# G-U-N/a-PyTorch-Tutorial-to-Class-Incremental-Learning

Measured on AMD Instinct MI355X. Metric: imgs/sec/node (CIFAR-100 B0-Inc10 ResNet-18 WA+KD step), higher is better.
Workload: dtype bf16; 1 GPU; model=resnet18, global_batch=128, input_size=32, kd=True, hip_graph=True, parallelism=dp1

## Files before the change

cilfw/_hip_ops.py:

```python

import ctypes
import os

import torch

_LIB_PATH = os.path.join(os.path.dirname(os.path.abspath(__file__)),
                         "_hip_lib.so")
if not os.path.exists(_LIB_PATH):
    raise ImportError(f"cilfw HIP library not built: {_LIB_PATH}")
_lib = ctypes.CDLL(_LIB_PATH)

_DEBUG = os.environ.get("CILFW_SYNC_DEBUG") == "1"

c_vp = ctypes.c_void_p
c_i = ctypes.c_int
c_l = ctypes.c_long
c_f = ctypes.c_float

_lib.cilfw_sync.restype = c_i
_lib.cilfw_error_string.restype = ctypes.c_char_p
_lib.cilfw_error_string.argtypes = [c_i]

_PROTOS = {
    "cilfw_conv2d_fwd": [c_vp] * 4 + [c_i] * 12 + [c_vp, c_vp],
    "cilfw_conv2d_bwd_data": [c_vp] * 4 + [c_i] * 12 + [c_vp] * 5 + [c_i, c_vp],
    "cilfw_conv2d_bwd_weight": [c_vp] * 5 + [c_i] * 13 + [c_vp],
    "cilfw_fill_mtable": [c_vp] + [c_i] * 4 + [c_vp],
    "cilfw_im2col_smallc": [c_vp] * 3 + [c_i] * 11 + [c_vp],
    "cilfw_bn_apply_only": [c_vp] * 7 + [c_l, c_i, c_i, c_vp],
    "cilfw_bn_fwd": [c_vp] * 11 + [c_i, c_l, c_i, c_f, c_f, c_i, c_i, c_vp],
    "cilfw_bn_bwd": [c_vp] * 11 + [c_vp, c_i] + [c_l, c_i, c_i, c_i, c_vp],
    "cilfw_add_relu_fwd": [c_vp] * 3 + [c_l, c_vp],
    "cilfw_add_relu_bwd": [c_vp] * 3 + [c_l, c_vp],
    "cilfw_downsample_a_fwd": [c_vp] * 2 + [c_i] * 4 + [c_vp],
    "cilfw_downsample_a_bwd": [c_vp] * 2 + [c_i] * 4 + [c_vp],
    "cilfw_gap_fwd": [c_vp] * 2 + [c_i] * 3 + [c_vp],
    "cilfw_gap_bwd": [c_vp] * 2 + [c_i] * 3 + [c_vp],
    "cilfw_conv2d_bwd_data_sub": [c_vp] * 4 + [c_i] * 12 + [c_vp],
    "cilfw_parity_scatter": [c_vp] * 2 + [c_i] * 8 + [c_vp],
    "cilfw_stride_gather": [c_vp] * 2 + [c_i] * 7 + [c_vp],
    "cilfw_stride_scatter": [c_vp] * 2 + [c_i] * 7 + [c_vp],
    "cilfw_maxpool_fwd": [c_vp] * 3 + [c_i] * 9 + [c_vp],
    "cilfw_maxpool_bwd": [c_vp] * 3 + [c_i] * 9 + [c_vp],
    "cilfw_linear_fwd": [c_vp] * 5 + [c_i] * 4 + [c_vp],
    "cilfw_linear_dx": [c_vp] * 4 + [c_i] * 4 + [c_vp],
    "cilfw_linear_dw": [c_vp] * 5 + [c_i] * 4 + [c_vp],
    "cilfw_ce_fwd": [c_vp] * 5 + [c_i, c_i, c_f, c_vp],
    "cilfw_ce_bwd": [c_vp] * 4 + [c_i, c_i, c_f, c_vp],
    "cilfw_kd_fwd": [c_vp] * 6 + [c_i, c_i, c_f, c_vp],
    "cilfw_kd_bwd": [c_vp] * 4 + [c_i, c_i, c_f, c_vp],
    "cilfw_wa_loss_fwd": [c_vp] * 8 + [c_i] * 3 + [c_f] * 3 + [c_vp],
    "cilfw_wa_loss_bwd": [c_vp] * 6 + [c_i] * 3 + [c_f] * 3 + [c_vp],
    "cilfw_sgd_step": [c_vp] * 4 + [c_l, c_vp, c_f, c_f, c_vp],
    "cilfw_topk_correct": [c_vp] * 3 + [c_i] * 3 + [c_vp],
    "cilfw_herding_select": [c_vp] * 3 + [c_i] * 3 + [c_vp],
    "cilfw_herding_select_batch": [c_vp] * 6 + [c_i] * 3 + [c_vp],
    "cilfw_crop_resize": [c_vp] * 7 + [c_i] * 7 + [c_vp],
    "cilfw_crop_resize_ragged": [c_vp] * 9 + [c_i] * 5 + [c_vp],
    "cilfw_nme_prototypes": [c_vp] * 3 + [c_i] * 2 + [c_vp],
    "cilfw_nme_topk": [c_vp] * 6 + [c_i] * 4 + [c_vp],
}
for _name, _args in _PROTOS.items():
    _fn = getattr(_lib, _name)
    _fn.argtypes = _args
    _fn.restype = None

_lib.cilfw_conv2d_bwd_data.restype = c_i

for _name, _n in [("cilfw_linear_ksplit", 3),
                  ("cilfw_conv2d_fwd_ksplit", 7),
                  ("cilfw_conv2d_bwd_data_ksplit", 7),
                  ("cilfw_conv2d_bwd_data_can_fuse_bn", 8),
                  ("cilfw_conv2d_bwd_data_bn_gy", 3),
                  ("cilfw_conv2d_bwd_weight_nslices", 7),
                  ("cilfw_conv2d_fwd_route", 8),
                  ("cilfw_conv2d_bwd_data_route", 9),
                  ("cilfw_conv2d_bwd_weight_route", 8)]:
    _fn = getattr(_lib, _name)
    _fn.argtypes = [c_i] * _n
    _fn.restype = c_i

_FWD_ROUTES = ("v1_bk32", "v1_bk64", "v2_bn64", "v2_bn128")
_BWD_DATA_ROUTES = ("s2_fused", "v2", "v1_bk32", "v1_bk64")
_BWD_WEIGHT_ROUTES = ("v2", "v1_fast", "v1_generic")


def _stream():
    return c_vp(torch.cuda.current_stream().cuda_stream)


# ... 47 lines not shown
        H, W_, stride = (H - 1) // stride + 1, (W_ - 1) // stride + 1, 1
    ks = _lib.cilfw_conv2d_bwd_data_ksplit(N, H, W_, C, K, R, S)
    return _BWD_DATA_ROUTES[_lib.cilfw_conv2d_bwd_data_route(
        N, H, W_, C, K, R, S, stride, ks)], ks


def _stem_im2col_dw(C, K, R, S):
    use_im2col = (os.environ.get("CILFW_STEM_IM2COL") == "1"
                  or (R * S >= 25
                      and os.environ.get("CILFW_STEM_IM2COL") != "0"))
    return C < 16 and R * S > 1 and K % 16 == 0 and use_im2col


def conv2d_bwd_weight_route(N, C, K, R, S, Ho, Wo, accum=False):
    if _stem_im2col_dw(C, K, R, S):
        N, C, R, S, Ho, Wo = N * Ho * Wo, (C * R * S + 15) // 16 * 16, 1, 1, \
            1, 1
        accum = False
    ns = _lib.cilfw_conv2d_bwd_weight_nslices(N, C, K, R, S, Ho, Wo)
    return _BWD_WEIGHT_ROUTES[_lib.cilfw_conv2d_bwd_weight_route(
        N, C, K, R, S, Ho, Wo, 1 if accum else 0)], ns


def conv2d_fwd(x, w, stride, pad, want_bn_parts=False):
    _bf16(x, "conv2d_fwd.x")
    _bf16(w, "conv2d_fwd.w")
    N, H, W_, C = x.shape
    R, S, Cw, K = w.shape
    assert Cw == C
    assert K % 8 == 0, "conv kernels vector-stage over output channels (K%8==0)"
    Ho = (H + 2 * pad - R) // stride + 1
    Wo = (W_ + 2 * pad - S) // stride + 1
    if C < 16 and R * S > 1 and K % 16 == 0 \
            and os.environ.get("CILFW_STEM_IM2COL") == "1":
        CRS = C * R * S
        CRSpad = (CRS + 15) // 16 * 16
        col, Ho, Wo = _stem_cols(x, stride, pad, R, S, CRSpad)
        M = N * Ho * Wo
        wpad = torch.zeros(CRSpad, K, dtype=torch.bfloat16, device=x.device)
        wpad[:CRS] = w.reshape(CRS, K)
        y = torch.empty(M, K, dtype=torch.bfloat16, device=x.device)
        ks = _lib.cilfw_conv2d_fwd_ksplit(M, CRSpad, K, 1, 1, 1, 1)
        ws = (torch.empty(ks * M * K, dtype=torch.float32, device=x.device)
              if ks > 1 else None)
        _lib.cilfw_conv2d_fwd(_ptr(col), _ptr(wpad), _ptr(y), _ptr(ws),
                              c_i(M), c_i(1), c_i(1), c_i(CRSpad), c_i(K),
                              c_i(1), c_i(1), c_i(1), c_i(0), c_i(1), c_i(1),
                              c_i(ks), _ptr(None), _stream())
        _check("conv2d_fwd_stem")
        return y.view(N, Ho, Wo, K), None
    y = torch.empty(N, Ho, Wo, K, dtype=torch.bfloat16, device=x.device)
    ks = _lib.cilfw_conv2d_fwd_ksplit(N, C, K, R, S, Ho, Wo)
    ws = (torch.empty(ks * N * Ho * Wo * K, dtype=torch.float32,
                      device=x.device) if ks > 1 else None)
    parts = None
    if want_bn_parts and ks == 1 \
            and _FWD_ROUTES[_lib.cilfw_conv2d_fwd_route(
                N, C, K, R, S, Ho, Wo, ks)].startswith("v2_") \
            and os.environ.get("CILFW_CONV_BN_FUSE", "1") != "0":
        gy = (N * Ho * Wo + 127) // 128
        parts = torch.empty(gy * 2 * K, dtype=torch.float32,
                            device=x.device)
    _lib.cilfw_conv2d_fwd(_ptr(x), _ptr(w), _ptr(y), _ptr(ws), c_i(N),
                          c_i(H), c_i(W_), c_i(C), c_i(K), c_i(R), c_i(S),
                          c_i(stride), c_i(pad), c_i(Ho), c_i(Wo), c_i(ks),
                          _ptr(parts), _stream())
    _check("conv2d_fwd")
    return y, parts


def conv2d_bwd_data(dy, w, stride, pad, H, W_, bn_meta=None):
    _bf16(dy, "conv2d_bwd_data.dy")
    N, Ho, Wo, K = dy.shape
    R, S, C, Kw = w.shape
    assert Kw == K
    if R == 1 and S == 1 and stride > 1:
        dxs = conv2d_bwd_data(dy, w, 1, 0, Ho, Wo)
        dx = torch.empty(N, H, W_, C, dtype=torch.bfloat16, device=dy.device)
        _lib.cilfw_stride_scatter(_ptr(dxs), _ptr(dx), c_i(N), c_i(H),
                                  c_i(W_), c_i(C), c_i(stride), c_i(Ho),
                                  c_i(Wo), _stream())
        _check("stride_scatter")
        return (dx, None) if bn_meta is not None else dx
    dx = torch.empty(N, H, W_, C, dtype=torch.bfloat16, device=dy.device)
    ks = _lib.cilfw_conv2d_bwd_data_ksplit(N, H, W_, C, K, R, S)
    ws = (torch.empty(ks * N * H * W_ * C, dtype=torch.float32,
                      device=dy.device) if ks > 1 else None)
    parts = None
    if (bn_meta is not None
            and _lib.cilfw_conv2d_bwd_data_can_fuse_bn(
                N, H, W_, C, K, R, S, stride)):
# ... 567 lines not shown
```

cilfw/csrc/common.h:

```cpp
#pragma once
#include <hip/hip_runtime.h>
#include <stdint.h>

#define WAVE 64
#define DEV __device__ __forceinline__

typedef __attribute__((ext_vector_type(8))) short bf16x8;
typedef __attribute__((ext_vector_type(4))) float f32x4;
typedef unsigned short bf16_t;

DEV float bf2f(bf16_t v) {
  union { uint32_t u; float f; } x;
  x.u = ((uint32_t)v) << 16;
  return x.f;
}

DEV bf16_t f2bf(float f) {
  union { uint32_t u; float f; } x;
  x.f = f;
  uint32_t u = x.u;
  uint32_t r = (u + 0x7fffu + ((u >> 16) & 1u)) >> 16;
  if ((u & 0x7f800000u) == 0x7f800000u && (u & 0x7fffffu)) r = (u >> 16) | 1u;
  return (bf16_t)r;
}

DEV int cdiv_i(int a, int b) { return (a + b - 1) / b; }
static inline int cdiv(int a, int b) { return (a + b - 1) / b; }

struct FragIdx {
  int half;
  int quad;
};
DEV FragIdx frag_idx() {
  int lane = threadIdx.x & (WAVE - 1);
  return {lane & 15, lane >> 4};
}
```

cilfw/csrc/conv.hip:

```cpp

#include "common.h"

#define BM 128
#define BN 64
#define NTHREADS 256

struct ConvGeom {
  int N, H, W, C, K, R, S, stride, pad, pad2, Ho, Wo;
  unsigned long long m_howo, m_wo;
  unsigned long long m_ck, m_s;
};

static inline unsigned long long magic40(int d) {
  return d > 0 ? ((1ULL << 40) / (unsigned)d + 1) : 0;
}

DEV unsigned mdiv40(unsigned n, unsigned long long m) {
  return (unsigned)(((unsigned long long)n * m) >> 40);
}

__global__ __launch_bounds__(NTHREADS)
void reduce_slabs_bf16_kernel(const float* __restrict__ ws,
                              bf16_t* __restrict__ out, int ns, long len) {
  long i0 = ((long)blockIdx.x * NTHREADS + threadIdx.x) * 4;
// ... 17 lines not shown

__global__ __launch_bounds__(NTHREADS)
void reduce_slabs_f32_kernel(const float* __restrict__ ws,
                             float* __restrict__ out, int ns, long len,
                             int accum) {
  long i0 = ((long)blockIdx.x * NTHREADS + threadIdx.x) * 4;
  if (i0 >= len) return;
  if (i0 + 4 <= len) {
    float4 acc = *(const float4*)&ws[i0];
    for (int s = 1; s < ns; ++s) {
      float4 v = *(const float4*)&ws[(long)s * len + i0];
      acc.x += v.x; acc.y += v.y; acc.z += v.z; acc.w += v.w;
    }
    if (accum) {
      float4 o = *(const float4*)&out[i0];
      acc.x += o.x; acc.y += o.y; acc.z += o.z; acc.w += o.w;
    }
    *(float4*)&out[i0] = acc;
  } else {
    for (long i = i0; i < len; ++i) {
      float a = ws[i];
      for (int s = 1; s < ns; ++s) a += ws[(long)s * len + i];
      out[i] = accum ? out[i] + a : a;
    }
  }
}


__device__ __forceinline__ int4 masked_i4(int4 v, bool ok) {
  int4 z{0, 0, 0, 0};
  return ok ? v : z;
}

template <int BKT, int BMX = BM, int BNX = BN, bool FAST = true>
__global__ __launch_bounds__(NTHREADS)
void conv2d_fwd_kernel(const bf16_t* __restrict__ x,
                       const bf16_t* __restrict__ w,
                       bf16_t* __restrict__ y, float* __restrict__ ws,
                       ConvGeom g, int M, int CRS, int nk, int fast_a,
                       int ksplit) {
  constexpr int NQ = BKT / 32;
  constexpr int LPX = BKT + 8;
  constexpr int NR = BMX / 128;
  constexpr int MR = BMX / 32;
  constexpr int NRC = BNX / 32;
  __shared__ bf16_t lds[2 * BMX * LPX + 2 * BNX * LPX];
// ... 794 lines not shown
  bf16_t* dst = &col[(long)m * CRSpad + rs * g.C];
  for (int c = 0; c < g.C; ++c) dst[c] = src[c];
}

__global__ __launch_bounds__(NTHREADS)
void fill_mtable_kernel(int* __restrict__ mt, int M, int HoWo, int Wo,
                        int stride) {
  int m = blockIdx.x * NTHREADS + threadIdx.x;
  if (m >= M) return;
  int n = m / HoWo;
  int rem = m - n * HoWo;
  int ho = rem / Wo;
  int wo = rem - ho * Wo;
  mt[m] = (n << 20) | ((ho * stride) << 10) | (wo * stride);
}



#define V2BK 64
#define V2_A_ELEMS (BM * V2BK)
#define V2_B_ELEMS (4 * V2BK * 16)
#define V2_BUF (V2_A_ELEMS + V2_B_ELEMS)

template <int BNX2 = BN>
__global__ __launch_bounds__(NTHREADS)
void conv2d_fwd_v2_kernel(const bf16_t* __restrict__ x,
                          const bf16_t* __restrict__ w,
                          bf16_t* __restrict__ y, float* __restrict__ ws,
                          const bf16_t* __restrict__ zpage, ConvGeom g,
                          int M, int CRS, int nk, int ksplit,
                          float* __restrict__ bn_parts) {
  constexpr int NGRP = BNX2 / 16;
  constexpr int NRC = BNX2 / 32;
  constexpr int BEL = NGRP * V2BK * 16;
  constexpr int BUFE = V2_A_ELEMS + BEL;
  __shared__ bf16_t lds[2 * BUFE];
  const int m0 = blockIdx.x * BM;
  const int n0 = blockIdx.y * BNX2;
  const int t = threadIdx.x;
  const int wv = t >> 6, lane = t & 63;
  const int wr = wv >> 1, wc = wv & 1;
  const int steps = (nk + ksplit - 1) / ksplit;
  const int kt0 = blockIdx.z * steps;
  const int kt1 = min(kt0 + steps, nk);
  const int nsteps = kt1 - kt0;

  int achunk[4], ar[4], as_[4], ac[4];
  bool mok[4];
  int an[4], ahb[4], awb[4];
#pragma unroll
  for (int i = 0; i < 4; ++i) {
    int row = wv * 32 + i * 8 + (lane >> 3);
    achunk[i] = (lane & 7) ^ (row & 7);
    int m = m0 + row;
// ... 90 lines not shown
    for (int q = 0; q < 2; ++q) {
      const int kb = fq * 8 + q * 32;
#pragma unroll
      for (int mr = 0; mr < 4; ++mr) {
        int row = wr * 64 + mr * 16 + fh;
        int kcol = kb ^ ((row & 7) << 3);
        bf16x8 afr = *(const bf16x8*)&As[row * V2BK + kcol];
        if (q == 0 && mr == 0) {
          asm volatile("s_waitcnt lgkmcnt(0)" ::: "memory");
          __builtin_amdgcn_sched_barrier(0);
          __builtin_amdgcn_s_setprio(1);
        }
#pragma unroll
        for (int nr = 0; nr < NRC; ++nr)
          acc[mr][nr] = __builtin_amdgcn_mfma_f32_16x16x32_bf16(
              afr, bfr[q][nr], acc[mr][nr], 0, 0, 0);
      }
    }
    __builtin_amdgcn_s_setprio(0);
    asm volatile("s_waitcnt vmcnt(0)" ::: "memory");
    __builtin_amdgcn_s_barrier();
  }

#pragma unroll
  for (int mr = 0; mr < 4; ++mr)
#pragma unroll
    for (int nr = 0; nr < NRC; ++nr)
#pragma unroll
      for (int r = 0; r < 4; ++r) {
        int row = m0 + wr * 64 + mr * 16 + fq * 4 + r;
        int col = n0 + wc * (16 * NRC) + nr * 16 + fh;
        if (row < M && col < g.K) {
          if (ksplit > 1)
            ws[((long)blockIdx.z * M + row) * g.K + col] = acc[mr][nr][r];
          else
            y[(long)row * g.K + col] = f2bf(acc[mr][nr][r]);
        }
      }

  if (bn_parts != nullptr) {
    __syncthreads();
    float* red = (float*)lds;
#pragma unroll
    for (int nr = 0; nr < NRC; ++nr) {
      float s1 = 0.f, s2 = 0.f;
#pragma unroll
      for (int mr = 0; mr < 4; ++mr)
#pragma unroll
        for (int r = 0; r < 4; ++r) {
          int row = m0 + wr * 64 + mr * 16 + fq * 4 + r;
          float v = (row < M) ? bf2f(f2bf(acc[mr][nr][r])) : 0.f;
          s1 += v;
          s2 += v * v;
        }
      int cl = wc * (16 * NRC) + nr * 16 + fh;
      red[((wv * 4 + fq) * BNX2 + cl) * 2] = s1;
// ... 415 lines not shown
      bn128 = e ? atoi(e) : 1;
    }
    static int min3x3 = -2;
    if (min3x3 == -2) {
      const char* e = getenv("CILFW_CONV_V2_BN128_MIN3X3");
      min3x3 = e ? atoi(e) : -1;
    }
    int shape_ok = (R == 1 && S == 1) || (min3x3 >= 0 && M >= min3x3);
    if (bn128 && K % 128 == 0 && shape_ok &&
        cdiv(M, BM) * cdiv(K, 128) * ksplit >= 256)
      return FWD_V2_BN128;
    return FWD_V2_BN64;
  }
  int use64 = bm == BM && (CRS >= bk64_min_crs()) &&
              (cdiv(M, BM) * cdiv(K, BN) * ksplit < bk64_max_blocks());
  return use64 ? FWD_V1_BK64 : FWD_V1_BK32;
}

int cilfw_conv2d_fwd_route(int N, int C, int K, int R, int S, int Ho, int Wo,
                           int ksplit) {
  return fwd_route(N * Ho * Wo, C, K, R, S, ksplit, 1);
}

void cilfw_conv2d_fwd(const void* x, const void* w, void* y, void* ws,
                      int N, int H, int W, int C, int K, int R, int S,
                      int stride, int pad, int Ho, int Wo, int ksplit,
                      void* bn_parts, void* stream) {
  ConvGeom g{N, H, W, C, K, R, S, stride, pad, pad, Ho, Wo,
             0, 0, magic40(C), magic40(S)};
  int M = N * Ho * Wo;
  int CRS = C * R * S;
  int fast_a = (C % 16 == 0);
  void* zp = fwd_v2_eligible(C) ? zpage_ptr() : nullptr;
  int route = fwd_route(M, C, K, R, S, ksplit, zp != nullptr);
  if (route == FWD_V2_BN128 || route == FWD_V2_BN64) {
    int nk2 = cdiv(CRS, V2BK);
    int bn2 = route == FWD_V2_BN128 ? 128 : BN;
    dim3 grid2(cdiv(M, BM), cdiv(K, bn2), ksplit);
    float* parts = (float*)(ksplit > 1 ? nullptr : bn_parts);
    if (route == FWD_V2_BN128)
      hipLaunchKernelGGL(conv2d_fwd_v2_kernel<128>, grid2, dim3(NTHREADS),
                         0, (hipStream_t)stream, (const bf16_t*)x,
                         (const bf16_t*)w, (bf16_t*)y, (float*)ws,
                         (const bf16_t*)zp, g, M, CRS, nk2, ksplit, parts);
    else
      hipLaunchKernelGGL(conv2d_fwd_v2_kernel<BN>, grid2, dim3(NTHREADS), 0,
                         (hipStream_t)stream, (const bf16_t*)x,
                         (const bf16_t*)w, (bf16_t*)y, (float*)ws,
                         (const bf16_t*)zp, g, M, CRS, nk2, ksplit, parts);
    if (ksplit > 1) {
      long len = (long)M * K;
      hipLaunchKernelGGL(reduce_slabs_bf16_kernel,
                         dim3((int)cdiv((long)len, (long)NTHREADS * 4)),
                         dim3(NTHREADS), 0, (hipStream_t)stream, (float*)ws,
                         (bf16_t*)y, ksplit, len);
    }
    return;
  }
  int bm = fwd_bm(M);
  int nk = cdiv(CRS, route == FWD_V1_BK64 ? 64 : 32);
  dim3 grid(cdiv(M, bm), cdiv(K, BN), ksplit);
#define LAUNCH_FWD(BKT_, BM_)                                                 \
  do {                                                                        \
    if (fast_a)                                                               \
      hipLaunchKernelGGL((conv2d_fwd_kernel<BKT_, BM_, BN, true>), grid,      \
                         dim3(NTHREADS), 0, (hipStream_t)stream,              \
                         (const bf16_t*)x, (const bf16_t*)w, (bf16_t*)y,      \
                         (float*)ws, g, M, CRS, nk, fast_a, ksplit);          \
    else                                                                      \
      hipLaunchKernelGGL((conv2d_fwd_kernel<BKT_, BM_, BN, false>), grid,     \
                         dim3(NTHREADS), 0, (hipStream_t)stream,              \
                         (const bf16_t*)x, (const bf16_t*)w, (bf16_t*)y,      \
                         (float*)ws, g, M, CRS, nk, fast_a, ksplit);          \
  } while (0)
  if (route == FWD_V1_BK64)
    LAUNCH_FWD(64, 128);
  else if (bm == 256)
    LAUNCH_FWD(32, 256);
  else
    LAUNCH_FWD(32, 128);
#undef LAUNCH_FWD
  if (ksplit > 1) {
    long len = (long)M * K;
    hipLaunchKernelGGL(reduce_slabs_bf16_kernel,
                       dim3((int)cdiv((long)len, (long)NTHREADS * 4)),
                       dim3(NTHREADS), 0, (hipStream_t)stream, (float*)ws,
                       (bf16_t*)y, ksplit, len);
  }
}

int cilfw_conv2d_fwd_ksplit(int N, int C, int K, int R, int S, int Ho,
                            int Wo) {
  int M = N * Ho * Wo;
  int CRS = C * R * S;
  int nk = cdiv(CRS, 32);
  return pick_ksplit(cdiv(M, BM) * cdiv(K, BN), nk);
}

static int bnbwd_fuse_enabled() {
  static int v = -1;
  if (v < 0) {
    const char* e = getenv("CILFW_BNBWD_FUSE");
    v = e ? atoi(e) : 0;
  }
  return v;
}

static int bwd_data_v2_eligible(int M, int K, int stride) {
  return K % 8 == 0 && stride <= 2 && conv_v2_enabled() &&
         M >= conv_v2_bwd_minm();
}
// ... 283 lines not shown
```

cilfw/csrc/norm.hip:

```cpp

#include "common.h"

#define NT 256


__global__ __launch_bounds__(NT)
void bn_sums_kernel(const bf16_t* __restrict__ x, float* __restrict__ part,
                    long M, int C, int rows_per_blk) {
  const int cg = threadIdx.x & 7;
  const int rl = threadIdx.x >> 3;
  const int c8 = blockIdx.x * 64 + cg * 8;
  const bool active = c8 + 8 <= C || c8 < C;
  long r0 = (long)blockIdx.y * rows_per_blk + rl;
  long r1 = min((long)(blockIdx.y + 1) * rows_per_blk, M);
  float s[8] = {0, 0, 0, 0, 0, 0, 0, 0};
  float q[8] = {0, 0, 0, 0, 0, 0, 0, 0};
  if (c8 + 8 <= C) {
    for (long r = r0; r < r1; r += 32) {
      int4 v = *(const int4*)&x[r * C + c8];
      const bf16_t* e = (const bf16_t*)&v;
#pragma unroll
      for (int j = 0; j < 8; ++j) {
        float f = bf2f(e[j]);
        s[j] += f;
// ... 88 lines not shown
    float mu = sum[c] / (float)M;
    float var = fmaxf(sumsq[c] / (float)M - mu * mu, 0.f);
    mean[c] = mu;
    invstd[c] = rsqrtf(var + eps);
    float unbiased = var * (float)M / (float)max(M - 1, 1L);
    running_mean[c] = (1.f - momentum) * running_mean[c] + momentum * mu;
    running_var[c] = (1.f - momentum) * running_var[c] + momentum * unbiased;
  } else {
    mean[c] = running_mean[c];
    invstd[c] = rsqrtf(running_var[c] + eps);
  }
}

__global__ __launch_bounds__(NT)
void bn_apply_kernel(const bf16_t* __restrict__ x, bf16_t* __restrict__ y,
                     const bf16_t* __restrict__ res,
                     const float* __restrict__ gamma,
                     const float* __restrict__ beta,
                     const float* __restrict__ mean,
                     const float* __restrict__ invstd,
                     long total, int C, int relu) {
  extern __shared__ float params[];
  for (int c = threadIdx.x; c < C; c += NT) {
    float sc = gamma[c] * invstd[c];
    params[c] = sc;
    params[C + c] = beta[c] - mean[c] * sc;
  }
  __syncthreads();
  long i0 = ((long)blockIdx.x * NT + threadIdx.x) * 8;
  if (i0 + 8 > total) {
    for (long i = i0; i < total; ++i) {
      int c = (int)(i % C);
      float v = bf2f(x[i]) * params[c] + params[C + c];
      if (res != nullptr) v += bf2f(res[i]);
      if (relu) v = fmaxf(v, 0.f);
      y[i] = f2bf(v);
    }
    return;
  }
  int4 xv = *(const int4*)&x[i0];
  bf16_t* xe = (bf16_t*)&xv;
  int4 rv;
  const bf16_t* re = (const bf16_t*)&rv;
  if (res != nullptr) rv = *(const int4*)&res[i0];
  bf16_t out[8];
  int c0 = (int)(i0 % C);
  float4 sc0 = *(const float4*)&params[c0];
  float4 sc1 = *(const float4*)&params[c0 + 4];
  float4 sh0 = *(const float4*)&params[C + c0];
  float4 sh1 = *(const float4*)&params[C + c0 + 4];
  float scv[8] = {sc0.x, sc0.y, sc0.z, sc0.w, sc1.x, sc1.y, sc1.z, sc1.w};
  float shv[8] = {sh0.x, sh0.y, sh0.z, sh0.w, sh1.x, sh1.y, sh1.z, sh1.w};
#pragma unroll
  for (int j = 0; j < 8; ++j) {
    float v = bf2f(xe[j]) * scv[j] + shv[j];
    if (res != nullptr) v += bf2f(re[j]);
    if (relu) v = fmaxf(v, 0.f);
    out[j] = f2bf(v);
  }
  *(int4*)&y[i0] = *(int4*)out;
}

__global__ __launch_bounds__(NT)
void bn_bwd_sums_kernel(const bf16_t* __restrict__ dy,
                        const bf16_t* __restrict__ x,
                        const bf16_t* __restrict__ y,
                        const float* __restrict__ mean,
                        const float* __restrict__ invstd,
                        float* __restrict__ part,
                        long M, int C, int rows_per_blk, int relu) {
  const int cg = threadIdx.x & 7;
  const int rl = threadIdx.x >> 3;
  const int c8 = blockIdx.x * 64 + cg * 8;
  float mu[8], is[8];
#pragma unroll
  for (int j = 0; j < 8; ++j) {
    int c = c8 + j;
    mu[j] = (c < C) ? mean[c] : 0.f;
    is[j] = (c < C) ? invstd[c] : 0.f;
  }
  long r0 = (long)blockIdx.y * rows_per_blk + rl;
// ... 607 lines not shown
```

cilfw/models/layers.py:

```python

import math

import torch
import torch.nn as nn

from ..ops import functional as CF


class Conv2d(nn.Module):

    def __init__(self, in_ch, out_ch, kernel_size, stride=1, padding=0):
        super().__init__()
        self.in_ch, self.out_ch = in_ch, out_ch
        self.kernel_size, self.stride, self.padding = kernel_size, stride, padding
        k = kernel_size
        self.weight = nn.Parameter(torch.empty(k, k, in_ch, out_ch))
        fan_in = k * k * in_ch
        nn.init.normal_(self.weight, 0.0, math.sqrt(2.0 / fan_in))

    def forward(self, x):
        return CF.conv2d(x, self.weight, self.stride, self.padding)

    def extra_repr(self):
        return (f"{self.in_ch}, {self.out_ch}, k={self.kernel_size}, "
# ... 12 lines not shown
        self.bias = nn.Parameter(torch.zeros(num_features))
        self.register_buffer("running_mean", torch.zeros(num_features))
        self.register_buffer("running_var", torch.ones(num_features))

    def forward(self, x, residual=None):
        assert not (self.training
                    and getattr(self.running_mean, "_cilfw_frozen", None)
                    is not None), \
            "BN has precomputed frozen eval stats but is in train mode"
        if residual is not None:
            return CF.batchnorm_add_relu(x, residual, self.weight, self.bias,
                                         self.running_mean, self.running_var,
                                         self.momentum, self.eps,
                                         self.training)
        return CF.batchnorm_act(x, self.weight, self.bias, self.running_mean,
                                self.running_var, self.momentum, self.eps,
                                self.training, self.relu,
                                fuse_bwd=self.fuse_bwd)

    def extra_repr(self):
        return f"{self.num_features}, relu={self.relu}"


class Linear(nn.Module):
    def __init__(self, in_features, out_features, bias=True):
        super().__init__()
        self.in_features, self.out_features = in_features, out_features
        self.weight = nn.Parameter(torch.empty(out_features, in_features))
        nn.init.kaiming_normal_(self.weight)
        if bias:
            self.bias = nn.Parameter(torch.zeros(out_features))
        else:
            self.register_parameter("bias", None)

    def forward(self, x):
        return CF.linear(x, self.weight, self.bias)

    def extra_repr(self):
        return f"{self.in_features}, {self.out_features}"
```

cilfw/models/resnet.py:

```python

import torch.nn as nn

from ..ops import functional as CF
from .layers import Conv2d, BatchNormAct2d


class BasicBlockB(nn.Module):
    expansion = 1

    def __init__(self, in_ch, out_ch, stride=1):
        super().__init__()
        self.conv1 = Conv2d(in_ch, out_ch, 3, stride=stride, padding=1)
        self.bn1 = BatchNormAct2d(out_ch, relu=True)
        self.conv2 = Conv2d(out_ch, out_ch, 3, stride=1, padding=1)
        self.bn2 = BatchNormAct2d(out_ch, relu=False)
        if stride != 1 or in_ch != out_ch:
            self.proj = Conv2d(in_ch, out_ch, 1, stride=stride, padding=0)
            self.proj_bn = BatchNormAct2d(out_ch, relu=False)
        else:
            self.proj = None

    def forward(self, x):
        out = self.bn1(self.conv1(x))
        residual = self.proj_bn(self.proj(x)) if self.proj is not None else x
        return self.bn2(self.conv2(out), residual)


class Bottleneck(nn.Module):
    expansion = 4

    def __init__(self, in_ch, width, stride=1):
        super().__init__()
        out_ch = width * self.expansion
        self.conv1 = Conv2d(in_ch, width, 1, stride=1, padding=0)
        self.bn1 = BatchNormAct2d(width, relu=True)
        self.conv2 = Conv2d(width, width, 3, stride=stride, padding=1)
        self.bn2 = BatchNormAct2d(width, relu=True)
        self.conv3 = Conv2d(width, out_ch, 1, stride=1, padding=0)
        self.bn3 = BatchNormAct2d(out_ch, relu=False)
        if stride != 1 or in_ch != out_ch:
            self.proj = Conv2d(in_ch, out_ch, 1, stride=stride, padding=0)
            self.proj_bn = BatchNormAct2d(out_ch, relu=False)
        else:
            self.proj = None

    def forward(self, x):
        out = self.bn1(self.conv1(x))
        out = self.bn2(self.conv2(out))
        residual = self.proj_bn(self.proj(x)) if self.proj is not None else x
        return self.bn3(self.conv3(out), residual)


class ResNet(nn.Module):
    def __init__(self, block, layers, in_channels=3, small_input=True):
        super().__init__()
        self.small_input = small_input
        if small_input:
            self.stem = Conv2d(in_channels, 64, 3, stride=1, padding=1)
        else:
            self.stem = Conv2d(in_channels, 64, 7, stride=2, padding=3)
        self.stem_bn = BatchNormAct2d(64, relu=True, fuse_bwd=False)
        self.in_ch = 64
        self.layer1 = self._make_layer(block, 64, layers[0], stride=1)
        self.layer2 = self._make_layer(block, 128, layers[1], stride=2)
        self.layer3 = self._make_layer(block, 256, layers[2], stride=2)
        self.layer4 = self._make_layer(block, 512, layers[3], stride=2)
        self.out_dim = 512 * block.expansion

    def _make_layer(self, block, width, n, stride):
        blocks = [block(self.in_ch, width, stride)]
        self.in_ch = width * block.expansion
        blocks += [block(self.in_ch, width, 1) for _ in range(n - 1)]
        return nn.Sequential(*blocks)

    def forward(self, x):
        x = self.stem_bn(self.stem(x))
        if not self.small_input:
            x = CF.max_pool(x, 3, 2, 1)
        x = self.layer1(x)
        x = self.layer2(x)
        x = self.layer3(x)
        x = self.layer4(x)
        return CF.global_avg_pool(x)


def resnet18(small_input=True, **kw):
    return ResNet(BasicBlockB, [2, 2, 2, 2], small_input=small_input, **kw)


def resnet34(small_input=True, **kw):
    return ResNet(BasicBlockB, [3, 4, 6, 3], small_input=small_input, **kw)


def resnet50(small_input=False, **kw):
    return ResNet(Bottleneck, [3, 4, 6, 3], small_input=small_input, **kw)
```

cilfw/models/resnet_cifar.py:

```python

import torch
import torch.nn as nn

from ..ops import functional as CF
from .layers import Conv2d, BatchNormAct2d


class BasicBlockA(nn.Module):

    def __init__(self, in_ch, out_ch, stride=1):
        super().__init__()
        self.conv_a = Conv2d(in_ch, out_ch, 3, stride=stride, padding=1)
        self.bn_a = BatchNormAct2d(out_ch, relu=True)
        self.conv_b = Conv2d(out_ch, out_ch, 3, stride=1, padding=1)
        self.bn_b = BatchNormAct2d(out_ch, relu=False)
        self.downsample = (stride != 1 or in_ch != out_ch)
        if self.downsample:
            assert stride == 2 and out_ch == 2 * in_ch, \
                "option-A downsample supports exactly stride2/double-channel"

    def forward(self, x):
        out = self.bn_a(self.conv_a(x))
        residual = CF.downsample_a(x) if self.downsample else x
        return self.bn_b(self.conv_b(out), residual)


class CifarResNet(nn.Module):

    def __init__(self, depth=32, in_channels=3):
        super().__init__()
        assert (depth - 2) % 6 == 0, "depth must be 6n+2"
        n = (depth - 2) // 6
        self.depth = depth
        self.conv_1_3x3 = Conv2d(in_channels, 16, 3, stride=1, padding=1)
        self.bn_1 = BatchNormAct2d(16, relu=True, fuse_bwd=False)
        self.stage_1 = self._make_stage(16, 16, n, stride=1)
        self.stage_2 = self._make_stage(16, 32, n, stride=2)
        self.stage_3 = self._make_stage(32, 64, n, stride=2)
        self.out_dim = 64

    @staticmethod
    def _make_stage(in_ch, out_ch, n, stride):
        blocks = [BasicBlockA(in_ch, out_ch, stride)]
        blocks += [BasicBlockA(out_ch, out_ch, 1) for _ in range(n - 1)]
        return nn.Sequential(*blocks)

    def forward(self, x):
        x = self.bn_1(self.conv_1_3x3(x))
        x = self.stage_1(x)
        x = self.stage_2(x)
        x = self.stage_3(x)
        return CF.global_avg_pool(x)


def resnet20(**kw):
    return CifarResNet(20, **kw)


def resnet32(**kw):
    return CifarResNet(32, **kw)


def resnet44(**kw):
    return CifarResNet(44, **kw)


def resnet56(**kw):
    return CifarResNet(56, **kw)


def resnet110(**kw):
# ... 2 lines not shown
```

cilfw/ops/functional.py:

```python

import torch
import torch.nn.functional as F

from ._backend import use_hip, ext


_wgrad_stream = None


def _wstream():
    global _wgrad_stream
    if _wgrad_stream is None:
        _wgrad_stream = torch.cuda.Stream()
    return _wgrad_stream


def _to_nchw(x):
    return x.permute(0, 3, 1, 2).contiguous()


def _to_nhwc(x):
    return x.permute(0, 2, 3, 1).contiguous()


# ... 21 lines not shown
    if parts is not None:
        dx._cilfw_bnbwd = (parts, bn_mean)
    return dx


class Conv2dNHWC(torch.autograd.Function):

    @staticmethod
    def forward(ctx, x, w, stride, padding, w_param=None):
        ctx.stride, ctx.padding = stride, padding
        if w_param is not None:
            w_param = w_param[0]
        wp = w_param if w_param is not None else w
        wc = getattr(wp, "_cilfw_bf16", None)
        if wc is None or wc.dtype != x.dtype:
            wc = w.to(x.dtype)
        ctx.save_for_backward(x, wc)
        ctx.w_dtype = w.dtype
        ctx.w_ref = wp
        ctx.sinked = w_param is not None
        ctx.bnbwd_src = getattr(x, "_cilfw_bnbwd_src", None)
        if use_hip(x):
            y, parts = ext().conv2d_fwd(x, wc, stride, padding,
                                        want_bn_parts=ctx.sinked)
            if parts is not None:
                y._cilfw_bn_parts = (parts, (y.numel() // y.shape[-1]
                                             + 127) // 128)
            return y
        xf = _to_nchw(x).float()
        wf = w.permute(3, 2, 0, 1).contiguous().float()
        y = F.conv2d(xf, wf, stride=stride, padding=padding)
        return _to_nhwc(y).to(x.dtype)

    @staticmethod
    def backward(ctx, dy):
        x, wc = ctx.saved_tensors
        stride, padding = ctx.stride, ctx.padding
        dy = dy.contiguous()
        need_dx = ctx.needs_input_grad[0]
        sink = getattr(ctx.w_ref, "_cilfw_sink", None) if ctx.sinked else None
        if use_hip(dy):
            R, S = wc.shape[0], wc.shape[1]
            cur = torch.cuda.current_stream()
            ws = _wstream()
            ws.wait_stream(cur)
            if sink is not None:
                eng, pi = sink
# ... 22 lines not shown
            dxf = torch.nn.grad.conv2d_input(xf.shape, wf, dyf, stride=stride,
                                             padding=padding)
            dx = _to_nhwc(dxf).to(x.dtype)
        dwf = torch.nn.grad.conv2d_weight(xf, wf.shape, dyf, stride=stride,
                                          padding=padding)
        dw = dwf.permute(2, 3, 1, 0).contiguous().to(ctx.w_dtype)
        if sink is not None:
            eng, pi = sink
            slot, accum = eng.sink_acquire(pi)
            out = slot.view_as(dw)
            (out.add_(dw) if accum else out.copy_(dw))
            eng.sink_delivered(pi)
            return dx, None, None, None, None
        return dx, dw, None, None, None


def conv2d(x, w, stride=1, padding=1):
    if (_sink_on() and x.requires_grad
            and getattr(w, "_cilfw_sink", None) is not None):
        return Conv2dNHWC.apply(x, w.detach(), stride, padding, [w])
    return Conv2dNHWC.apply(x, w, stride, padding)




def _gb_sinkable(x, gamma, beta):
    if not (_sink_on() and x.requires_grad):
        return False
    sg = getattr(gamma, "_cilfw_sink", None)
    sb = getattr(beta, "_cilfw_sink", None)
    return sg is not None and sb is not None and sg[0] is sb[0]


def _gb_deliver_hip(eng, gi, bi, bn_bwd_args, want_dres, ext_parts=None):
    gs, gacc = eng.sink_acquire(gi)
    bs, bacc = eng.sink_acquire(bi)
    if gacc or bacc:
        dx, dgamma, dbeta, dres = ext().bn_bwd(*bn_bwd_args,
                                               want_dres=want_dres,
                                               ext_parts=ext_parts)
        gs.add_(dgamma)
        bs.add_(dbeta)
    else:
        dx, _, _, dres = ext().bn_bwd(*bn_bwd_args, want_dres=want_dres,
                                      out_gamma=gs, out_beta=bs,
                                      ext_parts=ext_parts)
# ... 599 lines not shown
```

Baseline: 41720 imgs/s.

## Fuse frozen BN epilogue into conv forward and BN stats into split-K reduce

Adds a BN-apply epilogue (scale/shift, optional residual, ReLU) to the v2 conv forward kernel and a new split-K reduce kernel, used when a BatchNorm is frozen (eval mode, e.g. the KD teacher) and no grad is needed. It also lets split-K convs emit BN partial statistics from the reduce kernel instead of needing a separate stats pass. The aim is to remove separate BN-apply and stats kernel launches and the extra activation round-trips through memory. It adds template variants and a per-call fallback path, and partial sums are now computed from bf16-rounded values in the reduce.

```diff
diff --git a/cilfw/_hip_ops.py b/cilfw/_hip_ops.py
--- a/cilfw/_hip_ops.py
+++ b/cilfw/_hip_ops.py
@@ -22,7 +22,7 @@
 _lib.cilfw_error_string.argtypes = [c_i]
 
 _PROTOS = {
-    "cilfw_conv2d_fwd": [c_vp] * 4 + [c_i] * 12 + [c_vp, c_vp],
+    "cilfw_conv2d_fwd": [c_vp] * 4 + [c_i] * 12 + [c_vp] * 6 + [c_i, c_vp],
     "cilfw_conv2d_bwd_data": [c_vp] * 4 + [c_i] * 12 + [c_vp] * 5 + [c_i, c_vp],
     "cilfw_conv2d_bwd_weight": [c_vp] * 5 + [c_i] * 13 + [c_vp],
     "cilfw_fill_mtable": [c_vp] + [c_i] * 4 + [c_vp],
@@ -66,6 +66,8 @@
     _fn.restype = None
 
 _lib.cilfw_conv2d_bwd_data.restype = c_i
+_lib.cilfw_conv2d_fwd.restype = c_i
+_FWD_DID_BN_PARTS, _FWD_DID_BN_TAIL = 1, 2
 
 for _name, _n in [("cilfw_linear_ksplit", 3),
                   ("cilfw_conv2d_fwd_ksplit", 7),
@@ -159,7 +161,11 @@
         N, C, K, R, S, Ho, Wo, 1 if accum else 0)], ns
 
 
-def conv2d_fwd(x, w, stride, pad, want_bn_parts=False):
+def _conv_bn_tail_on():
+    return os.environ.get("CILFW_CONV_BN_TAIL", "1") != "0"
+
+
+def _conv2d_fwd(x, w, stride, pad, want_bn_parts, split_k_parts, bn_tail):
     _bf16(x, "conv2d_fwd.x")
     _bf16(w, "conv2d_fwd.w")
     N, H, W_, C = x.shape
@@ -183,27 +189,68 @@
         _lib.cilfw_conv2d_fwd(_ptr(col), _ptr(wpad), _ptr(y), _ptr(ws),
                               c_i(M), c_i(1), c_i(1), c_i(CRSpad), c_i(K),
                               c_i(1), c_i(1), c_i(1), c_i(0), c_i(1), c_i(1),
-                              c_i(ks), _ptr(None), _stream())
+                              c_i(ks), *([_ptr(None)] * 6), c_i(0), _stream())
         _check("conv2d_fwd_stem")
-        return y.view(N, Ho, Wo, K), None
+        return y.view(N, Ho, Wo, K), None, False
     y = torch.empty(N, Ho, Wo, K, dtype=torch.bfloat16, device=x.device)
     ks = _lib.cilfw_conv2d_fwd_ksplit(N, C, K, R, S, Ho, Wo)
     ws = (torch.empty(ks * N * Ho * Wo * K, dtype=torch.float32,
                       device=x.device) if ks > 1 else None)
     parts = None
-    if want_bn_parts and ks == 1 \
-            and _FWD_ROUTES[_lib.cilfw_conv2d_fwd_route(
-                N, C, K, R, S, Ho, Wo, ks)].startswith("v2_") \
+    if want_bn_parts and bn_tail is None \
             and os.environ.get("CILFW_CONV_BN_FUSE", "1") != "0":
-        gy = (N * Ho * Wo + 127) // 128
-        parts = torch.empty(gy * 2 * K, dtype=torch.float32,
-                            device=x.device)
-    _lib.cilfw_conv2d_fwd(_ptr(x), _ptr(w), _ptr(y), _ptr(ws), c_i(N),
-                          c_i(H), c_i(W_), c_i(C), c_i(K), c_i(R), c_i(S),
-                          c_i(stride), c_i(pad), c_i(Ho), c_i(Wo), c_i(ks),
-                          _ptr(parts), _stream())
+        if ks == 1:
+            fuse = _FWD_ROUTES[_lib.cilfw_conv2d_fwd_route(
+                N, C, K, R, S, Ho, Wo, ks)].startswith("v2_")
+        else:
+            fuse = split_k_parts and _conv_bn_tail_on()
+        if fuse:
+            gy = (N * Ho * Wo + 127) // 128
+            parts = torch.empty(gy * 2 * K, dtype=torch.float32,
+                                device=x.device)
+    tail = [_ptr(None)] * 5 + [c_i(0)]
+    if bn_tail is not None:
+        gamma, beta, mean, invstd, residual, relu = bn_tail
+        for t in (gamma, beta, mean, invstd):
+            assert t.dtype == torch.float32 and t.is_contiguous() \
+                and t.numel() == K, "conv2d_fwd: BN tail vectors are fp32 [K]"
+        if residual is not None:
+            _bf16(residual, "conv2d_fwd.residual")
+            assert residual.shape == y.shape
+        tail = [_ptr(gamma), _ptr(beta), _ptr(mean), _ptr(invstd),
+                _ptr(residual), c_i(1 if relu else 0)]
+    did = _lib.cilfw_conv2d_fwd(_ptr(x), _ptr(w), _ptr(y), _ptr(ws), c_i(N),
+                                c_i(H), c_i(W_), c_i(C), c_i(K), c_i(R),
+                                c_i(S), c_i(stride), c_i(pad), c_i(Ho),
+                                c_i(Wo), c_i(ks), _ptr(parts), *tail,
+                                _stream())
     _check("conv2d_fwd")
+    if not did & _FWD_DID_BN_PARTS:
+        parts = None
+    return y, parts, bool(did & _FWD_DID_BN_TAIL)
+
+
+def conv2d_fwd(x, w, stride, pad, want_bn_parts=False, split_k_parts=False):
+    y, parts, _ = _conv2d_fwd(x, w, stride, pad, want_bn_parts,
+                              split_k_parts, None)
     return y, parts
+
+
+def conv2d_bn_frozen_fwd(x, w, stride, pad, gamma, beta, mean, invstd,
+                         residual=None, relu=False):
+    gf = gamma.float().contiguous()
+    bf = beta.float().contiguous()
+    y, _, applied = _conv2d_fwd(x, w, stride, pad, False, False,
+                                (gf, bf, mean, invstd, residual, relu))
+    if applied:
+        return y
+    out = torch.empty_like(y)
+    _lib.cilfw_bn_apply_only(_ptr(y), _ptr(out), _ptr(residual), _ptr(gf),
+                             _ptr(bf), _ptr(mean), _ptr(invstd),
+                             c_l(y.numel()), c_i(y.shape[-1]),
+                             c_i(1 if relu else 0), _stream())
+    _check("bn_apply_only")
+    return out
 
 
 def conv2d_bwd_data(dy, w, stride, pad, H, W_, bn_meta=None):
diff --git a/cilfw/csrc/common.h b/cilfw/csrc/common.h
--- a/cilfw/csrc/common.h
+++ b/cilfw/csrc/common.h
@@ -24,6 +24,29 @@
   return (bf16_t)r;
 }
 
+DEV void bn_fold(float gamma, float invstd, float beta, float mean,
+                 float& sc, float& sh) {
+  sc = gamma * invstd;
+  sh = beta - mean * sc;
+}
+
+DEV float bn_affine(float x, float sc, float sh, bool has_res, float res,
+                    int relu) {
+  float v = x * sc + sh;
+  if (has_res) v += res;
+  if (relu) v = fmaxf(v, 0.f);
+  return v;
+}
+
+struct BnTail {
+  const float* gamma;
+  const float* beta;
+  const float* mean;
+  const float* invstd;
+  const bf16_t* res;
+  int relu;
+};
+
 DEV int cdiv_i(int a, int b) { return (a + b - 1) / b; }
 static inline int cdiv(int a, int b) { return (a + b - 1) / b; }
 
diff --git a/cilfw/csrc/conv.hip b/cilfw/csrc/conv.hip
--- a/cilfw/csrc/conv.hip
+++ b/cilfw/csrc/conv.hip
@@ -63,6 +63,91 @@
       float a = ws[i];
       for (int s = 1; s < ns; ++s) a += ws[(long)s * len + i];
       out[i] = accum ? out[i] + a : a;
+    }
+  }
+}
+
+enum { RSBN_STATS = 0, RSBN_APPLY = 1 };
+
+template <int MODE>
+__global__ __launch_bounds__(NTHREADS)
+void reduce_slabs_bn_kernel(const float* __restrict__ ws,
+                            bf16_t* __restrict__ out, int ns, int M, int K,
+                            float* __restrict__ parts, BnTail bt) {
+  const int cg = threadIdx.x & 15;
+  const int rl = threadIdx.x >> 4;
+  const int m0 = blockIdx.x * 128;
+  const int col = blockIdx.y * 64 + cg * 4;
+  const bool cok = col < K;
+  const int colc = cok ? col : 0;
+  const long slab = (long)M * K;
+  long idx[8];
+  float4 acc[8];
+#pragma unroll
+  for (int p = 0; p < 8; ++p) {
+    int row = min(m0 + p * 16 + rl, M - 1);
+    idx[p] = (long)row * K + colc;
+    acc[p] = *(const float4*)&ws[idx[p]];
+  }
+  for (int s = 1; s < ns; ++s) {
+    const float* w = ws + (long)s * slab;
+#pragma unroll
+    for (int p = 0; p < 8; ++p) {
+      float4 v = *(const float4*)&w[idx[p]];
+      acc[p].x += v.x; acc[p].y += v.y; acc[p].z += v.z; acc[p].w += v.w;
+    }
+  }
+  if (MODE == RSBN_STATS) {
+    float s1[4] = {0.f, 0.f, 0.f, 0.f}, s2[4] = {0.f, 0.f, 0.f, 0.f};
+#pragma unroll
+    for (int p = 0; p < 8; ++p) {
+      const bool ok = cok && (m0 + p * 16 + rl < M);
+      float a[4] = {acc[p].x, acc[p].y, acc[p].z, acc[p].w};
+      bf16_t o[4];
+#pragma unroll
+      for (int j = 0; j < 4; ++j) {
+        o[j] = f2bf(a[j]);
+        float v = ok ? bf2f(o[j]) : 0.f;
+        s1[j] += v;
+        s2[j] += v * v;
+      }
+      if (ok) *(int2*)&out[idx[p]] = *(int2*)o;
+    }
+    __shared__ float red[2][16][64];
+#pragma unroll
+    for (int j = 0; j < 4; ++j) {
+      red[0][rl][cg * 4 + j] = s1[j];
+      red[1][rl][cg * 4 + j] = s2[j];
+    }
+    __syncthreads();
+    if (threadIdx.x < 128) {
+      const int q = threadIdx.x >> 6, c = threadIdx.x & 63;
+      float a = 0.f;
+#pragma unroll
+      for (int r = 0; r < 16; ++r) a += red[q][r][c];
+      if (blockIdx.y * 64 + c < K)
+        parts[((long)blockIdx.x * 2 + q) * K + blockIdx.y * 64 + c] = a;
+    }
+  } else {
+    float sc[4], sh[4];
+#pragma unroll
+    for (int j = 0; j < 4; ++j)
+      bn_fold(bt.gamma[colc + j], bt.invstd[colc + j], bt.beta[colc + j],
+              bt.mean[colc + j], sc[j], sh[j]);
+    const bool has_res = bt.res != nullptr;
+#pragma unroll
+    for (int p = 0; p < 8; ++p) {
+      const bool ok = cok && (m0 + p * 16 + rl < M);
+      float a[4] = {acc[p].x, acc[p].y, acc[p].z, acc[p].w};
+      int2 rv{0, 0};
+      if (has_res) rv = *(const int2*)&bt.res[idx[p]];
+      const bf16_t* re = (const bf16_t*)&rv;
+      bf16_t o[4];
+#pragma unroll
+      for (int j = 0; j < 4; ++j)
+        o[j] = f2bf(bn_affine(bf2f(f2bf(a[j])), sc[j], sh[j], has_res,
+                              bf2f(re[j]), bt.relu));
+      if (ok) *(int2*)&out[idx[p]] = *(int2*)o;
     }
   }
 }
@@ -903,14 +988,14 @@
 #define V2_B_ELEMS (4 * V2BK * 16)
 #define V2_BUF (V2_A_ELEMS + V2_B_ELEMS)
 
-template <int BNX2 = BN>
+template <int BNX2 = BN, bool TAIL = false>
 __global__ __launch_bounds__(NTHREADS)
 void conv2d_fwd_v2_kernel(const bf16_t* __restrict__ x,
                           const bf16_t* __restrict__ w,
                           bf16_t* __restrict__ y, float* __restrict__ ws,
                           const bf16_t* __restrict__ zpage, ConvGeom g,
                           int M, int CRS, int nk, int ksplit,
-                          float* __restrict__ bn_parts) {
+                          float* __restrict__ bn_parts, BnTail bt) {
   constexpr int NGRP = BNX2 / 16;
   constexpr int NRC = BNX2 / 32;
   constexpr int BEL = NGRP * V2BK * 16;
@@ -1047,6 +1132,15 @@
     __builtin_amdgcn_s_barrier();
   }
 
+  float tsc[NRC], tsh[NRC];
+  if (TAIL) {
+#pragma unroll
+    for (int nr = 0; nr < NRC; ++nr) {
+      int cc = min(n0 + wc * (16 * NRC) + nr * 16 + fh, g.K - 1);
+      bn_fold(bt.gamma[cc], bt.invstd[cc], bt.beta[cc], bt.mean[cc],
+              tsc[nr], tsh[nr]);
+    }
+  }
 #pragma unroll
   for (int mr = 0; mr < 4; ++mr)
 #pragma unroll
@@ -1056,7 +1150,11 @@
         int row = m0 + wr * 64 + mr * 16 + fq * 4 + r;
         int col = n0 + wc * (16 * NRC) + nr * 16 + fh;
         if (row < M && col < g.K) {
-          if (ksplit > 1)
+          if (TAIL)
+            y[(long)row * g.K + col] = f2bf(bn_affine(
+                bf2f(f2bf(acc[mr][nr][r])), tsc[nr], tsh[nr], false, 0.f,
+                bt.relu));
+          else if (ksplit > 1)
             ws[((long)blockIdx.z * M + row) * g.K + col] = acc[mr][nr][r];
           else
             y[(long)row * g.K + col] = f2bf(acc[mr][nr][r]);
@@ -1518,15 +1616,49 @@
   return fwd_route(N * Ho * Wo, C, K, R, S, ksplit, 1);
 }
 
-void cilfw_conv2d_fwd(const void* x, const void* w, void* y, void* ws,
-                      int N, int H, int W, int C, int K, int R, int S,
-                      int stride, int pad, int Ho, int Wo, int ksplit,
-                      void* bn_parts, void* stream) {
+enum { FWD_DID_BN_PARTS = 1, FWD_DID_BN_TAIL = 2 };
+
+static int launch_fwd_reduce(const float* ws, bf16_t* y, int ksplit, int M,
+                             int K, float* bn_parts, const BnTail& bt,
+                             hipStream_t st) {
+  const int tail_ok = (K % 4 == 0);
+  if (tail_ok && (bt.mean != nullptr || bn_parts != nullptr)) {
+    dim3 grid(cdiv(M, 128), cdiv(K, 64));
+    if (bt.mean != nullptr) {
+      hipLaunchKernelGGL(reduce_slabs_bn_kernel<RSBN_APPLY>, grid,
+                         dim3(NTHREADS), 0, st, ws, y, ksplit, M, K,
+                         (float*)nullptr, bt);
+      return FWD_DID_BN_TAIL;
+    }
+    hipLaunchKernelGGL(reduce_slabs_bn_kernel<RSBN_STATS>, grid,
+                       dim3(NTHREADS), 0, st, ws, y, ksplit, M, K, bn_parts,
+                       bt);
+    return FWD_DID_BN_PARTS;
+  }
+  long len = (long)M * K;
+  hipLaunchKernelGGL(reduce_slabs_bf16_kernel,
+                     dim3((int)cdiv((long)len, (long)NTHREADS * 4)),
+                     dim3(NTHREADS), 0, st, ws, y, ksplit, len);
+  return 0;
+}
+
+int cilfw_conv2d_fwd(const void* x, const void* w, void* y, void* ws,
+                     int N, int H, int W, int C, int K, int R, int S,
+                     int stride, int pad, int Ho, int Wo, int ksplit,
+                     void* bn_parts, const void* bn_gamma,
+                     const void* bn_beta, const void* bn_mean,
+                     const void* bn_invstd, const void* bn_res, int bn_relu,
+                     void* stream) {
   ConvGeom g{N, H, W, C, K, R, S, stride, pad, pad, Ho, Wo,
              0, 0, magic40(C), magic40(S)};
   int M = N * Ho * Wo;
   int CRS = C * R * S;
   int fast_a = (C % 16 == 0);
+  hipStream_t st = (hipStream_t)stream;
+  BnTail bt{(const float*)bn_gamma, (const float*)bn_beta,
+            (const float*)bn_mean, (const float*)bn_invstd,
+            (const bf16_t*)bn_res, bn_relu};
+  const BnTail no_tail{nullptr, nullptr, nullptr, nullptr, nullptr, 0};
   void* zp = fwd_v2_eligible(C) ? zpage_ptr() : nullptr;
   int route = fwd_route(M, C, K, R, S, ksplit, zp != nullptr);
   if (route == FWD_V2_BN128 || route == FWD_V2_BN64) {
@@ -1534,24 +1666,24 @@
     int bn2 = route == FWD_V2_BN128 ? 128 : BN;
     dim3 grid2(cdiv(M, BM), cdiv(K, bn2), ksplit);
     float* parts = (float*)(ksplit > 1 ? nullptr : bn_parts);
-    if (route == FWD_V2_BN128)
-      hipLaunchKernelGGL(conv2d_fwd_v2_kernel<128>, grid2, dim3(NTHREADS),
-                         0, (hipStream_t)stream, (const bf16_t*)x,
-                         (const bf16_t*)w, (bf16_t*)y, (float*)ws,
-                         (const bf16_t*)zp, g, M, CRS, nk2, ksplit, parts);
-    else
-      hipLaunchKernelGGL(conv2d_fwd_v2_kernel<BN>, grid2, dim3(NTHREADS), 0,
-                         (hipStream_t)stream, (const bf16_t*)x,
-                         (const bf16_t*)w, (bf16_t*)y, (float*)ws,
-                         (const bf16_t*)zp, g, M, CRS, nk2, ksplit, parts);
-    if (ksplit > 1) {
-      long len = (long)M * K;
-      hipLaunchKernelGGL(reduce_slabs_bf16_kernel,
-                         dim3((int)cdiv((long)len, (long)NTHREADS * 4)),
-                         dim3(NTHREADS), 0, (hipStream_t)stream, (float*)ws,
-                         (bf16_t*)y, ksplit, len);
-    }
-    return;
+    const int tail = ksplit == 1 && bt.mean != nullptr && bt.res == nullptr;
+#define LAUNCH_FWD_V2(BN_, TAIL_)                                             \
+  hipLaunchKernelGGL((conv2d_fwd_v2_kernel<BN_, TAIL_>), grid2,               \
+                     dim3(NTHREADS), 0, st, (const bf16_t*)x,                 \
+                     (const bf16_t*)w, (bf16_t*)y, (float*)ws,                \
+                     (const bf16_t*)zp, g, M, CRS, nk2, ksplit,               \
+                     TAIL_ ? (float*)nullptr : parts, TAIL_ ? bt : no_tail)
+    if (route == FWD_V2_BN128) {
+      if (tail) LAUNCH_FWD_V2(128, true); else LAUNCH_FWD_V2(128, false);
+    } else {
+      if (tail) LAUNCH_FWD_V2(BN, true); else LAUNCH_FWD_V2(BN, false);
+    }
+#undef LAUNCH_FWD_V2
+    if (ksplit > 1)
+      return launch_fwd_reduce((const float*)ws, (bf16_t*)y, ksplit, M, K,
+                               (float*)bn_parts, bt, st);
+    if (tail) return FWD_DID_BN_TAIL;
+    return parts != nullptr ? FWD_DID_BN_PARTS : 0;
   }
   int bm = fwd_bm(M);
   int nk = cdiv(CRS, route == FWD_V1_BK64 ? 64 : 32);
@@ -1560,12 +1692,12 @@
   do {                                                                        \
     if (fast_a)                                                               \
       hipLaunchKernelGGL((conv2d_fwd_kernel<BKT_, BM_, BN, true>), grid,      \
-                         dim3(NTHREADS), 0, (hipStream_t)stream,              \
+                         dim3(NTHREADS), 0, st,                               \
                          (const bf16_t*)x, (const bf16_t*)w, (bf16_t*)y,      \
                          (float*)ws, g, M, CRS, nk, fast_a, ksplit);          \
     else                                                                      \
       hipLaunchKernelGGL((conv2d_fwd_kernel<BKT_, BM_, BN, false>), grid,     \
-                         dim3(NTHREADS), 0, (hipStream_t)stream,              \
+                         dim3(NTHREADS), 0, st,                               \
                          (const bf16_t*)x, (const bf16_t*)w, (bf16_t*)y,      \
                          (float*)ws, g, M, CRS, nk, fast_a, ksplit);          \
   } while (0)
@@ -1576,13 +1708,10 @@
   else
     LAUNCH_FWD(32, 128);
 #undef LAUNCH_FWD
-  if (ksplit > 1) {
-    long len = (long)M * K;
-    hipLaunchKernelGGL(reduce_slabs_bf16_kernel,
-                       dim3((int)cdiv((long)len, (long)NTHREADS * 4)),
-                       dim3(NTHREADS), 0, (hipStream_t)stream, (float*)ws,
-                       (bf16_t*)y, ksplit, len);
-  }
+  if (ksplit > 1)
+    return launch_fwd_reduce((const float*)ws, (bf16_t*)y, ksplit, M, K,
+                             (float*)bn_parts, bt, st);
+  return 0;
 }
 
 int cilfw_conv2d_fwd_ksplit(int N, int C, int K, int R, int S, int Ho,
diff --git a/cilfw/csrc/norm.hip b/cilfw/csrc/norm.hip
--- a/cilfw/csrc/norm.hip
+++ b/cilfw/csrc/norm.hip
@@ -134,19 +134,19 @@
                      long total, int C, int relu) {
   extern __shared__ float params[];
   for (int c = threadIdx.x; c < C; c += NT) {
-    float sc = gamma[c] * invstd[c];
+    float sc, sh;
+    bn_fold(gamma[c], invstd[c], beta[c], mean[c], sc, sh);
     params[c] = sc;
-    params[C + c] = beta[c] - mean[c] * sc;
+    params[C + c] = sh;
   }
   __syncthreads();
   long i0 = ((long)blockIdx.x * NT + threadIdx.x) * 8;
   if (i0 + 8 > total) {
     for (long i = i0; i < total; ++i) {
       int c = (int)(i % C);
-      float v = bf2f(x[i]) * params[c] + params[C + c];
-      if (res != nullptr) v += bf2f(res[i]);
-      if (relu) v = fmaxf(v, 0.f);
-      y[i] = f2bf(v);
+      y[i] = f2bf(bn_affine(bf2f(x[i]), params[c], params[C + c],
+                            res != nullptr,
+                            res != nullptr ? bf2f(res[i]) : 0.f, relu));
     }
     return;
   }
@@ -165,10 +165,8 @@
   float shv[8] = {sh0.x, sh0.y, sh0.z, sh0.w, sh1.x, sh1.y, sh1.z, sh1.w};
 #pragma unroll
   for (int j = 0; j < 8; ++j) {
-    float v = bf2f(xe[j]) * scv[j] + shv[j];
-    if (res != nullptr) v += bf2f(re[j]);
-    if (relu) v = fmaxf(v, 0.f);
-    out[j] = f2bf(v);
+    out[j] = f2bf(bn_affine(bf2f(xe[j]), scv[j], shv[j], res != nullptr,
+                            res != nullptr ? bf2f(re[j]) : 0.f, relu));
   }
   *(int4*)&y[i0] = *(int4*)out;
 }
diff --git a/cilfw/models/layers.py b/cilfw/models/layers.py
--- a/cilfw/models/layers.py
+++ b/cilfw/models/layers.py
@@ -58,6 +58,15 @@
         return f"{self.num_features}, relu={self.relu}"
 
 
+def conv_bn(conv, bn, x, residual=None):
+    if CF.conv_bn_frozen_ok(x, conv.weight, bn, residual):
+        return CF.conv_bn_frozen(x, conv.weight, conv.stride, conv.padding,
+                                 bn, residual,
+                                 relu=True if residual is not None
+                                 else bn.relu)
+    return bn(conv(x), residual)
+
+
 class Linear(nn.Module):
     def __init__(self, in_features, out_features, bias=True):
         super().__init__()
diff --git a/cilfw/models/resnet.py b/cilfw/models/resnet.py
--- a/cilfw/models/resnet.py
+++ b/cilfw/models/resnet.py
@@ -2,7 +2,7 @@
 import torch.nn as nn
 
 from ..ops import functional as CF
-from .layers import Conv2d, BatchNormAct2d
+from .layers import Conv2d, BatchNormAct2d, conv_bn
 
 
 class BasicBlockB(nn.Module):
@@ -21,9 +21,10 @@
             self.proj = None
 
     def forward(self, x):
-        out = self.bn1(self.conv1(x))
-        residual = self.proj_bn(self.proj(x)) if self.proj is not None else x
-        return self.bn2(self.conv2(out), residual)
+        out = conv_bn(self.conv1, self.bn1, x)
+        residual = conv_bn(self.proj, self.proj_bn, x) \
+            if self.proj is not None else x
+        return conv_bn(self.conv2, self.bn2, out, residual)
 
 
 class Bottleneck(nn.Module):
@@ -45,10 +46,11 @@
             self.proj = None
 
     def forward(self, x):
-        out = self.bn1(self.conv1(x))
-        out = self.bn2(self.conv2(out))
-        residual = self.proj_bn(self.proj(x)) if self.proj is not None else x
-        return self.bn3(self.conv3(out), residual)
+        out = conv_bn(self.conv1, self.bn1, x)
+        out = conv_bn(self.conv2, self.bn2, out)
+        residual = conv_bn(self.proj, self.proj_bn, x) \
+            if self.proj is not None else x
+        return conv_bn(self.conv3, self.bn3, out, residual)
 
 
 class ResNet(nn.Module):
@@ -74,7 +76,7 @@
         return nn.Sequential(*blocks)
 
     def forward(self, x):
-        x = self.stem_bn(self.stem(x))
+        x = conv_bn(self.stem, self.stem_bn, x)
         if not self.small_input:
             x = CF.max_pool(x, 3, 2, 1)
         x = self.layer1(x)
diff --git a/cilfw/models/resnet_cifar.py b/cilfw/models/resnet_cifar.py
--- a/cilfw/models/resnet_cifar.py
+++ b/cilfw/models/resnet_cifar.py
@@ -3,7 +3,7 @@
 import torch.nn as nn
 
 from ..ops import functional as CF
-from .layers import Conv2d, BatchNormAct2d
+from .layers import Conv2d, BatchNormAct2d, conv_bn
 
 
 class BasicBlockA(nn.Module):
@@ -20,9 +20,9 @@
                 "option-A downsample supports exactly stride2/double-channel"
 
     def forward(self, x):
-        out = self.bn_a(self.conv_a(x))
+        out = conv_bn(self.conv_a, self.bn_a, x)
         residual = CF.downsample_a(x) if self.downsample else x
-        return self.bn_b(self.conv_b(out), residual)
+        return conv_bn(self.conv_b, self.bn_b, out, residual)
 
 
 class CifarResNet(nn.Module):
@@ -46,7 +46,7 @@
         return nn.Sequential(*blocks)
 
     def forward(self, x):
-        x = self.bn_1(self.conv_1_3x3(x))
+        x = conv_bn(self.conv_1_3x3, self.bn_1, x)
         x = self.stage_1(x)
         x = self.stage_2(x)
         x = self.stage_3(x)
diff --git a/cilfw/ops/functional.py b/cilfw/ops/functional.py
--- a/cilfw/ops/functional.py
+++ b/cilfw/ops/functional.py
@@ -67,7 +67,8 @@
         ctx.bnbwd_src = getattr(x, "_cilfw_bnbwd_src", None)
         if use_hip(x):
             y, parts = ext().conv2d_fwd(x, wc, stride, padding,
-                                        want_bn_parts=ctx.sinked)
+                                        want_bn_parts=ctx.sinked,
+                                        split_k_parts=True)
             if parts is not None:
                 y._cilfw_bn_parts = (parts, (y.numel() // y.shape[-1]
                                              + 127) // 128)
@@ -136,6 +137,29 @@
     return Conv2dNHWC.apply(x, w, stride, padding)
 
 
+def conv_bn_frozen_ok(x, w, bn_module, residual=None):
+    import os
+    if os.environ.get("CILFW_CONV_BN_TAIL", "1") == "0" or not use_hip(x):
+        return False
+    if bn_module.training or getattr(bn_module.running_mean, "_cilfw_frozen",
+                                     None) is None:
+        return False
+    if not torch.is_grad_enabled():
+        return True
+    ts = (x, w, bn_module.weight, bn_module.bias, residual)
+    return not any(t is not None and t.requires_grad for t in ts)
+
+
+def conv_bn_frozen(x, w, stride, padding, bn_module, residual=None,
+                   relu=False):
+    mean, invstd = bn_module.running_mean._cilfw_frozen
+    wc = w if w.dtype == x.dtype else w.to(x.dtype)
+    with torch.no_grad():
+        return ext().conv2d_bn_frozen_fwd(
+            x, wc, stride, padding, bn_module.weight, bn_module.bias, mean,
+            invstd, residual=residual, relu=relu)
+
+
 
 
 def _gb_sinkable(x, gamma, beta):
```

Measured after the change: 42180 imgs/s (median of 4 runs). No clear change (+1.1%).
